# tzjtatata/Myriad

Hardware: AMD Instinct MI355X
Metric: images/sec fine-tune step (Vicuna-7B + LoRA-style adapters, 224px) (higher is better)
Workload: dtype bf16

## Files before the change

include/myriad_hip.h:

```cpp
#ifndef MYRIAD_HIP_H
#define MYRIAD_HIP_H
#include <stdint.h>

#ifdef __cplusplus
extern "C" {
#endif

typedef struct ihipStream_t* mh_stream_t;

#define MH_OK 0
#define MH_ERR_ARG (-1)
#define MH_ERR_LAUNCH (-2)
#define MH_ERR_UNSUPPORTED (-3)

#define MH_GEMM_OUT_F32 1
#define MH_GEMM_GELU 2
#define MH_GEMM_REGSTAGE 4

int mh_gemm_bf16_nt(const void* A, int lda, const void* B, int ldb, void* C, int ldc, int M, int N, int K,
                    const float* bias, const float* residual, int ldr, int flags, float alpha, mh_stream_t s);

int mh_gemm_plan(int M, int N, int K, int flags, int* kernel, int* splits);

int mh_prof_start(int capacity, mh_stream_t s);
// ... 57 lines not shown
long mh_layernorm_param_grads_ws_floats(int M, int D);
int mh_layernorm_param_grads(const float* dy, const float* x, float* dgamma, float* dbeta, int M, int D, float eps,
                             int accumulate, float p_out, unsigned long long seed_out, float* ws, long ws_floats,
                             mh_stream_t s);
int mh_layernorm_fwd_dropout(const float* z, const float* res, const float* w, const float* b, float* x_out, void* y_bf16,
                             float* y_f32, int M, int D, float eps, float p_in, unsigned long long seed_in, float p_out,
                             unsigned long long seed_out, mh_stream_t s);
int mh_layernorm_bwd_dropout(const float* dy, const float* x, const float* w, float* dx, void* dz_bf16, int M, int D,
                             float eps, float p_in, unsigned long long seed_in, float p_out, unsigned long long seed_out,
                             mh_stream_t s);
int mh_dropout_keep_mask(float* out, long n, float p, unsigned long long seed, mh_stream_t s);
long mh_gemm_tn_wgrad_ws_floats(int M, int N, int K, int splits);
int mh_gemm_tn_wgrad_auto_splits(int M, int N, int K);
int mh_gemm_tn_wgrad(const void* dy, long lddy, const void* x, long ldx, float* out, long ldo, float* bias, int M, int N, int K,
                     int accumulate, int splits, float* ws, long ws_floats, mh_stream_t s);

int mh_rope_inplace(void* x, int ld, int col0, int n_tok, int n_heads, int head_dim, const int* pos,
                    const float* cos_tab, const float* sin_tab, float sign, mh_stream_t s);
int mh_silu_mul_fwd(const void* gu, void* h, int M, int I, mh_stream_t s);
int mh_silu_mul_bwd(const void* dh, const void* gu, void* dgu, int M, int I, mh_stream_t s);
int mh_silu_mul_fwd_blk(const void* gu, void* h, int M, int I, int blk, mh_stream_t s);
int mh_silu_mul_bwd_blk(const void* dh, const void* gu, void* dgu, int M, int I, int blk, mh_stream_t s);
int mh_gemm_swiglu_fwd(const void* X, int ldx, const void* Wgu, int ldw, void* gu, int ldgu, void* act, int ldact, int M,
                       int I, int K, mh_stream_t s);
int mh_gemm_swiglu_bwd(const void* dH, int lddh, const void* WdT, int ldw, const void* gu, int ldgu, void* dgu, int lddgu,
                       void* dact_buf, int M, int I, int K, mh_stream_t s);
int mh_gelu_fwd(const void* x, void* y, long n, mh_stream_t s);
int mh_gelu_bwd(const void* dy, const void* x, void* dx, long n, mh_stream_t s);
int mh_gemm_gelu_fwd(const void* X, int ldx, const void* W, int ldw, const float* bias, void* pre, int ldpre, void* act, int ldact,
                     int M, int N, int K, mh_stream_t s);
// ... 205 lines not shown
                        const void* eroded, int y0s, int x0s, int dy0, int dx0, int h, int w, const double* Sh, const double* cy,
                        const double* Sw, const double* cx, double* ws, int mixed, mh_stream_t s);

int mh_adamw_gated(float* p, const float* g, float* m, float* v, long n, double lr, double beta1, double beta2, double eps,
                   double weight_decay, double grad_scale, const float* used, const int* steps, mh_stream_t s);
int mh_adamw_bump(const float* used, int* steps, int n, mh_stream_t s);

long mh_grad_sumsq_slots(long n);
int mh_grad_sumsq(const float* g, long n, const float* used, double* partials, long slots, mh_stream_t s);
int mh_clip_rank_sum(const double* partials, long n_partials, double* rank_sums, int world, int rank, mh_stream_t s);
int mh_clip_finalize(const double* partials, long n_partials, const double* rank_sums, int world, double max_norm,
                     double grad_scale, int guard, double* ctl, mh_stream_t s);
int mh_adamw_gated_ctl(float* p, const float* g, float* m, float* v, long n, double lr, double beta1, double beta2, double eps,
                       double weight_decay, const float* used, const int* steps, const double* ctl, mh_stream_t s);
int mh_adamw_bump_ctl(const float* used, int* steps, int n, const double* ctl, mh_stream_t s);

int mh_l2norm_rows(const float* x, long ldx, void* y_bf16, float* y_f32, long ldy, int M, int D, float eps, mh_stream_t s);
int mh_pair_logits(const float* p, long ldp, const float* text, float* out, long rows, int rows_per_batch, int C, float scale,
                   mh_stream_t s);
int mh_zs_accumulate(const float* logits, float* mask_acc, float* map_acc, int B, int h, int S, float w, mh_stream_t s);
int mh_rowmax_skip(const float* scores, long lds, float* acc, long rows, int cols, int period, float w, mh_stream_t s);
int mh_bilinear_ac(const float* in, float* out, int B, int h, int w, int H, int W, int one_minus, mh_stream_t s);

int mh_bank_sim_chunk_rows(void);
int mh_bank_sim_max(const void* q, long q_row0, long q_sample_rows, const void* bank, const int* bank_off, const int* bank_rows,
                    float* part, int B, int L, int D, int max_chunks, mh_stream_t s);
int mh_bank_sim_finish(const float* part, const int* bank_rows, float* sim, float* simmask, float* amap, int T, int B,
                       int max_chunks, int h, int S, float w, mh_stream_t s);

long mh_mask_components_lds_bytes(int H, int W);
// ... 37 lines not shown
```

myriad_amd/csrc/optim.hip:

```cpp
#include "common.h"

__global__ void adamw_kernel(float* __restrict__ p, const float* __restrict__ g, float* __restrict__ m,
                             float* __restrict__ v, bf16_t* __restrict__ shadow, long n4, float lr, float beta1,
                             float beta2, float omb1, float omb2, float eps, float wd, float bc1, float bc2_sqrt,
                             float gscale) {
  for (long it = blockIdx.x * (long)blockDim.x + threadIdx.x; it < n4; it += (long)gridDim.x * blockDim.x) {
    float4_t pp = *reinterpret_cast<const float4_t*>(p + it * 4);
    const float4_t gg = *reinterpret_cast<const float4_t*>(g + it * 4);
    float4_t mm = *reinterpret_cast<const float4_t*>(m + it * 4);
    float4_t vv = *reinterpret_cast<const float4_t*>(v + it * 4);
#pragma unroll
    for (int e = 0; e < 4; ++e) {
      const float gr = gg[e] * gscale;
      pp[e] *= (1.f - lr * wd);
      mm[e] = beta1 * mm[e] + omb1 * gr;
      vv[e] = beta2 * vv[e] + omb2 * gr * gr;
      const float denom = sqrtf(vv[e]) / bc2_sqrt + eps;
      pp[e] -= (lr / bc1) * (mm[e] / denom);
    }
    *reinterpret_cast<float4_t*>(p + it * 4) = pp;
    *reinterpret_cast<float4_t*>(m + it * 4) = mm;
    *reinterpret_cast<float4_t*>(v + it * 4) = vv;
    if (shadow) {
      uint2 pk;
// ... 218 lines not shown
  if (ctl[2] != 0.0 && i < n && used[i] > 0.f) steps[i] += 1;
}

extern "C" int mh_adamw_gated_ctl(float* p, const float* g, float* m, float* v, long n, double lr, double beta1, double beta2,
                                  double eps, double weight_decay, const float* used, const int* steps, const double* ctl,
                                  hipStream_t stream) {
  if (n < 0 || n % 4 || !used || !steps || !ctl || (n > 0 && (!p || !g || !m || !v))) return MH_ERR_ARG;
  if (n == 0) return MH_OK;
  long grid = (n / 4 + 255) / 256;
  if (grid > 256 * 16) grid = 256 * 16;
  hipLaunchKernelGGL(adamw_gated_ctl_kernel, dim3((int)grid), dim3(256), 0, stream, p, g, m, v, n / 4, (float)lr, beta1, beta2,
                     (float)eps, (float)weight_decay, used, steps, ctl);
  MH_CHECK_LAUNCH();
  return MH_OK;
}
extern "C" int mh_adamw_bump_ctl(const float* used, int* steps, int n, const double* ctl, hipStream_t stream) {
  if (n <= 0) return MH_OK;
  if (!used || !steps || !ctl) return MH_ERR_ARG;
  hipLaunchKernelGGL(adamw_bump_ctl_kernel, dim3((n + 63) / 64), dim3(64), 0, stream, used, steps, n, ctl);
  MH_CHECK_LAUNCH();
  return MH_OK;
}
```

myriad_amd/csrc/wgrad.hip:

```cpp
#include "common.h"

#define TN_BN 64
#define TN_BK 64
#define TN_BM 32
#define TN_RS (TN_BK + 16)
typedef __attribute__((address_space(3))) short4_t tn_lds_s4;

__device__ __forceinline__ short8_t tn_frag(const bf16_t* img, int jd, int lr, int lg) {
  const bf16_t* p = img + (4 * lg + (lr >> 2)) * TN_RS + 16 * jd + 4 * (lr & 3);
  const short4_t a = __builtin_amdgcn_ds_read_tr16_b64_v4i16((tn_lds_s4*)p);
  const short4_t b = __builtin_amdgcn_ds_read_tr16_b64_v4i16((tn_lds_s4*)(p + 16 * TN_RS));
  return (short8_t){a[0], a[1], a[2], a[3], b[0], b[1], b[2], b[3]};
}

__global__ __launch_bounds__(256) void gemm_tn_wgrad_kernel(const bf16_t* __restrict__ dy, long lddy, const bf16_t* __restrict__ x,
                                                            long ldx, float* out, long ldo, float* bias, float* ws, float* wsb,
                                                            int M, int N, int K, int rows_per, int accumulate) {
  __shared__ __attribute__((aligned(16))) bf16_t img[2][TN_BM * TN_RS];
  __shared__ float red[TN_BM][TN_BN + 1];
  const int tid = threadIdx.x, lane = tid & 63, wave = tid >> 6, lr = lane & 15, lg = lane >> 4;
  const int k0 = blockIdx.x * TN_BK, n0 = blockIdx.y * TN_BN, z = blockIdx.z;
  const int m0 = z * rows_per;
  const int m1 = min(M, m0 + rows_per);
  const bool want_bias = bias != nullptr && blockIdx.x == 0;
// ... 109 lines not shown
  rows_per = (rows_per + TN_BM - 1) / TN_BM * TN_BM;
  if (rows_per == 0) rows_per = TN_BM;
  float* wsb = splits > 1 ? ws + (long)splits * N * K : nullptr;
  hipLaunchKernelGGL(gemm_tn_wgrad_kernel, dim3(K / TN_BK, N / TN_BN, splits), dim3(256), 0, stream, (const bf16_t*)dy, lddy,
                     (const bf16_t*)x, ldx, out, ldo, bias, ws, wsb, M, N, K, rows_per, accumulate);
  MH_CHECK_LAUNCH();
  if (splits > 1) {
    const long n4 = (long)N * (K / 4);
    hipLaunchKernelGGL(tn_split_reduce_kernel, dim3((unsigned)((n4 + 255) / 256)), dim3(256), 0, stream, ws, wsb, splits, out,
                       ldo, bias, N, K, accumulate);
    MH_CHECK_LAUNCH();
  }
  return MH_OK;
}

#define LNP_NT 256
#define LNP_NW 4
#define LNP_ROWS 16
#define LNP_IT 4

__global__ __launch_bounds__(LNP_NT) void layernorm_param_partial_kernel(const float* __restrict__ dy, const float* __restrict__ x,
                                                                         float* __restrict__ part, int M, int D, float eps,
                                                                         float p_out, unsigned long long seed_out) {
  __shared__ float red[LNP_NW];
  const int r0 = blockIdx.x * LNP_ROWS, r1 = min(M, r0 + LNP_ROWS);
  float4_t sg[LNP_IT], sb[LNP_IT];
#pragma unroll
  for (int c = 0; c < LNP_IT; ++c) sg[c] = sb[c] = (float4_t){0.f, 0.f, 0.f, 0.f};
  for (int row = r0; row < r1; ++row) {
    const float* xr = x + (size_t)row * D;
// ... 83 lines not shown
```

myriad_amd/myriad.py:

```python
from __future__ import annotations

import numbers
import os
import random
from collections import OrderedDict
from typing import Dict, List, Optional, Tuple

import torch
import torch.nn as nn

from . import _lib, ops
from .eva_vit import EvaViTHIP
from .llama import LlamaHIP
from .networks import LoraAdaptor, VENet, from_reference_layout, to_reference_layout, ve_param_specs
from .qformer import QFormerHIP, qformer_param_specs
from .registry import registry

BF16, F32 = torch.bfloat16, torch.float32


def uses_weight_decay(name: str, ndim: int) -> bool:
    return not (ndim < 2 or "bias" in name or "ln" in name or "bn" in name)


# ... 97 lines not shown
        self.steps_dev = torch.zeros(max(nm, 1), dtype=torch.int32, device=self.dev)
        self.flat_m = torch.zeros(off, dtype=F32, device=self.dev)
        self.flat_v = torch.zeros(off, dtype=F32, device=self.dev)
        self.p, self.g = {}, {}
        self.ref_shape = {}
        for name, ishape, rshape in self.specs:
            o, n = self.offsets[name]
            self.p[name] = self.flat_p[o:o + n].view(ishape)
            self.g[name] = self.flat_g[o:o + n].view(ishape)
            self.ref_shape[name] = rshape
        self.ctl = None
        self._norm_ws = None
        self._rank_sums = None
        self.step = 0
        self.version = 0

    def n_params(self) -> int:
        return sum(n for _, n in self.offsets.values())

    def mark_used(self, used_modules) -> None:
        if not self.modules:
            return
        flags = torch.tensor([1.0 if m in used_modules else 0.0 for m in self.modules], dtype=F32)
        self.used.copy_(ops.h2d(flags, self.dev))

    def module_steps(self) -> Dict[str, int]:
        st = self.steps_dev.cpu().tolist()
        return {m: int(st[i]) for i, m in enumerate(self.modules)}

    def set_module_steps(self, steps: Dict[str, int]) -> None:
# ... 2 lines not shown

    def module_range(self, module: str, decays: bool = True):
        if module not in self.modules:
            return None
        mi = self.modules.index(module)
        for m2, a, b, d in self.ranges:
            if m2 == mi and d == decays:
                return a, b
        return None

    def adamw_module(self, module: str, lr: float, weight_decay: float = 0.05, beta2: float = 0.999) -> None:
        mi = self.modules.index(module)
        self.version += 1
        for m2, a, b, decays in self.ranges:
            if m2 == mi:
                ops.adamw_gated(self.flat_p[a:b], self.flat_g[a:b], self.flat_m[a:b], self.flat_v[a:b], lr,
                                weight_decay if decays else 0.0, self.used[mi:mi + 1], self.steps_dev[mi:mi + 1], beta2=beta2)

    def adamw_pieces(self, pieces, lr: float, weight_decay: float = 0.05, beta2: float = 0.999, grad_scale: float = 1.0) -> None:
        self.version += 1
        for mi, a0, b0, decays in self.ranges:
            for lo, hi in pieces:
                a, b = max(a0, lo), min(b0, hi)
                if a < b:
                    ops.adamw_gated(self.flat_p[a:b], self.flat_g[a:b], self.flat_m[a:b], self.flat_v[a:b], lr,
                                    weight_decay if decays else 0.0, self.used[mi:mi + 1], self.steps_dev[mi:mi + 1], beta2=beta2,
                                    grad_scale=grad_scale)

    def adamw_step(self, lr: float, weight_decay: float = 0.05, beta2: float = 0.999, grad_scale: float = 1.0, shard=None,
                   skip=(), exclude=(), clip=None):
        self.step += 1
        self.version += 1
        pieces = None
        if shard is not None:
            pieces = [tuple(shard)] if isinstance(shard[0], int) else [tuple(p) for p in shard]
            if sum(hi - lo for lo, hi in pieces) < self.total:
                self.moments_complete = False
        skip_idx = {self.modules.index(m) for m in skip if m in self.modules}
        todo = update_pieces(self.ranges, pieces, exclude, skip_idx)
        if clip is not None:
            self._prepare_clip(todo, grad_scale, clip)
        for mi, a, b, decays in todo:
            if clip is None:
                ops.adamw_gated(self.flat_p[a:b], self.flat_g[a:b], self.flat_m[a:b], self.flat_v[a:b], lr,
                                weight_decay if decays else 0.0, self.used[mi:mi + 1], self.steps_dev[mi:mi + 1], beta2=beta2,
                                grad_scale=grad_scale)
            else:
                ops.adamw_gated_ctl(self.flat_p[a:b], self.flat_g[a:b], self.flat_m[a:b], self.flat_v[a:b], lr,
                                    weight_decay if decays else 0.0, self.used[mi:mi + 1], self.steps_dev[mi:mi + 1], self.ctl,
                                    beta2=beta2)
        if self.modules:
            if clip is None:
                ops.adamw_bump(self.used, self.steps_dev)
            else:
                ops.adamw_bump_ctl(self.used, self.steps_dev, self.ctl)

    def _prepare_clip(self, todo, grad_scale: float, clip) -> None:
        if self.ctl is None:
            self.ctl = torch.zeros(4, dtype=torch.float64, device=self.dev)
        need = sum(ops.grad_sumsq_slots(b - a) for _, a, b, _ in todo)
        if self._norm_ws is None or self._norm_ws.numel() < need:
            whole = sum(ops.grad_sumsq_slots(b - a) for _, a, b, _ in self.ranges)
            self._norm_ws = torch.zeros(max(need, whole) + 64, dtype=torch.float64, device=self.dev)
        ws, off = self._norm_ws, 0
        for mi, a, b, _ in todo:
# ... 31 lines not shown
            fan_in = cin * k * k
        bound = 1.0 / math.sqrt(fan_in)
        return (torch.rand(rshape) * 2 - 1) * bound
    raise KeyError(f"{name}: not in the weight files and no constructor init exists (load it with `ckpt`)")


class _LossBridge(torch.autograd.Function):

    @staticmethod
    def forward(ctx, anchor, model, loss):
        ctx.model = model
        return loss.detach().clone()

    @staticmethod
    def backward(ctx, gout):
        ctx.model.backward(float(gout), accumulate=ctx.model._grads_live())
        return None, None, None


class MyriadHIP(nn.Module):
    arch = "myriad"

    def __init__(self, weights, cfg: Optional[dict] = None, device="cuda:0"):
        super().__init__()
        cfg = dict(cfg or {})
        self.cfg = cfg
        self._dev = torch.device(device)
        self.max_txt_len = cfg.get("max_txt_len", 160)
        self.end_sym = cfg.get("end_sym", "###")
        self.k_shot = cfg.get("k_shot", 0)
# ... 56 lines not shown
        self._params = OrderedDict()
        for name, ishape, rshape in self.store.specs:
            if name in lora_init and name not in weights:
                src = lora_init[name]
            elif name in weights:
                src = weights[name]
            else:
                src = init_trainable(name, rshape)
            self.store.p[name].copy_(from_reference_layout(src.to(self._dev, F32), ishape))
            prm = nn.Parameter(self.store.p[name], requires_grad=True)
            prm.grad = self.store.g[name]
            self._params[name] = prm
            self._register_dotted(name, prm)
        if self.arch == "myriad":
            self.adaptor = LoraAdaptor(self.store.p, self.store.g)
            self.ve_tok = VENet("VETokenizer.", 5, self.Dl, self.store.p, self.store.g, self._dev)
            self.ve_ins = VENet("VEInstructor.", 1, self.Dq, self.store.p, self.store.g, self._dev)
        if self.use_lora:
            self.lora = LoraQV(len(self.llama.layers), self.Dl, int(cfg.get("lora_r", 8)),
                               float(cfg.get("lora_alpha", 16)), float(cfg.get("lora_dropout", 0.05)),
                               self.store.p, self.store.g, self._dev)
            self.lora.base_seed = int(cfg.get("lora_dropout_seed", torch.initial_seed())) & ((1 << 31) - 1)
            self.llama.attach_lora(self.lora)
        if self.train_qformer:
            self.query_tokens_f32 = self.store.p["query_tokens"]
            self.qformer.bind_trainable(self.store, need_denc=self.arch == "myriad" or self.train_vit)
        if self.train_vit:
            self.ln_w, self.ln_b = self.store.p["ln_vision.weight"], self.store.p["ln_vision.bias"]
            self.vit.bind_trainable(self.store, need_backward=need_bwd)
        self._pending_update = None
        self._vit_stream, self._vit_prefetched = None, None
# ... 42 lines not shown
    def merged_lora_state_dict(self) -> "OrderedDict[str, torch.Tensor]":
        if not self.use_lora:
            raise ValueError("merged_lora_state_dict: no LoRA is attached (cfg use_lora)")
        from .lora import merged_qv_names
        self.finish_update()
        out, D = OrderedDict(), self.Dl
        for i, L in enumerate(self.llama.layers):
            m = self.lora.merge_layer(i, L, "rows")
            nq, nv = merged_qv_names(i)
            out[nq], out[nv] = m[:D].clone(), m[2 * D:].clone()
        return out

    def load_state_dict(self, sd, strict: bool = False):
        self.finish_update()
        self.store.version += 1
        missing = []
        for name, ishape, _ in self.store.specs:
            if name in sd:
                self.store.p[name].copy_(from_reference_layout(sd[name].to(self._dev, F32), ishape))
            else:
                missing.append(name)
        if self.train_vit:
            self.vit.refresh()
        else:
            self._load_vision_keys(sd)
        if strict and missing:
            raise KeyError(missing)
        return missing

    @torch.no_grad()
# ... 243 lines not shown
        if c is None:
            raise RuntimeError("backward() without a training forward")
        head = None
        if accumulate and float(gscale) == 1.0 and self.arch == "myriad" and self.ve_tok.head_accumulates_in_place:
            o_n = self.store.offsets.get("VETokenizer.meta_net.15.weight")
            if o_n is not None and o_n[1] >= (1 << 20):
                head = (o_n[0], o_n[0] + o_n[1])
        self._acc_head = head
        fg = self.store.flat_g_comm
        if not accumulate:
            prev = None
        elif head is None:
            prev = fg.clone()
        else:
            prev = (fg[:head[0]].clone(), fg[head[1]:].clone())
        zeroed, self._g_zeroed = getattr(self, "_g_zeroed", None), None
        if zeroed is not None and not accumulate:
            torch.cuda.current_stream().wait_event(zeroed)
        elif head is None:
            fg.zero_()
        else:
            fg[:head[0]].zero_()
            fg[head[1]:].zero_()
        used = {"lora"} if self.use_lora else set()
        if self.arch == "myriad":
            used.add("expert_adaptor")
            if c["use_tok"]:
                used.add("VETokenizer")
            if c["use_ins"]:
                used.add("VEInstructor")
        else:
            used.add("llama_proj")
        if self.train_qformer:
            used.add("Qformer")
        if self.train_vit:
            used.update(("visual_encoder", "ln_vision"))
        self.store.mark_used(used)
        self._bridge_used = (self._bridge_used | used) if accumulate else set(used)
# ... 65 lines not shown
            else:
                self.ve_ins.backward(dins)
        dy = self._ln_vision_backward(denc, c)
        dx = self.adaptor.backward(dy, need_dx=self.train_vit)
        if self.train_vit:
            self.vit.backward(dx.view(B, c["N"], self.Dv), grads=self.vit.grad_views)
        if self.llama.lora is not None:
            self.llama.lora.join_wgrads()
        if leaf_ev is not None:
            torch.cuda.current_stream().wait_event(leaf_ev)
        if ins_ev is not None:
            torch.cuda.current_stream().wait_event(ins_ev)
        del leaf_keep, ins_keep
        self._finish_backward()

    def _ln_vision_backward(self, denc: torch.Tensor, c) -> torch.Tensor:
        d2 = denc.view(c["B"] * c["N"], self.Dv)
        if self.train_vit:
            ops.layernorm_param_grads(d2, c["y"], 1e-5, self.store.g["ln_vision.weight"], self.store.g["ln_vision.bias"])
        return ops.layernorm_bwd(d2, c["y"], self.ln_w, 1e-5)[0]

    def _query_tokens_grad(self, dq: torch.Tensor) -> None:
        B, nq, D = dq.shape
        self.store.g["query_tokens"].view(-1).copy_(ops.colsum(dq.reshape(B, nq * D)[:, :self.nq0 * D]))

    def _start_early_exchange(self, early_exchange) -> None:
        dp, k = early_exchange[0], early_exchange[1]
        st = self.store
        if len(early_exchange) > 2 and getattr(dp, "supports_early_update", False):
            lr, wd, beta2 = early_exchange[2]

            def then():
                st.adamw_pieces(dp.part_shards(st.total, k), lr, wd, beta2=beta2, grad_scale=1.0 / dp.world)
                dp.gather_part(st.flat_p, k)
            dp.start_part(st.flat_g_comm, st.total, k, then=then)
        else:
            dp.start_part(st.flat_g_comm, st.total, k)

    def _finish_backward(self):
        if self._bwd_gscale != 1.0:
            ops.scale_(self.store.flat_g, self._bwd_gscale)
        if self._bwd_prev is not None:
            fg = self.store.flat_g_comm
            if isinstance(self._bwd_prev, tuple):
                a, b = self._acc_head
                for pv, dst in ((self._bwd_prev[0], fg[:a]), (self._bwd_prev[1], fg[b:])):
                    if pv.numel():
                        ops.copy2d(pv.view(1, -1), dst.view(1, -1), accumulate=True)
            else:
# ... 112 lines not shown
            vit_out = self._take_prefetched_vit(samples)
            if next_samples is not None:
                self.prefetch_vit(next_samples)
            if self._pending_update is not None and vit_out is not None:
                self.finish_update()
            elif self._pending_update is not None and self.train_vit:
                self.finish_update()
            elif self._pending_update is not None:
                vit_out = self.vit.forward(self._image_of(samples))
                self.finish_update()
            if (self._accum_count == 0 and self._leaf_aside and self._dev.type == "cuda"
                    and os.environ.get("MYRIAD_EARLY_ZERO", "1") != "0"):
                aux, main = self._side_stream("leaf"), torch.cuda.current_stream()
                aux.wait_stream(main)
                with torch.cuda.stream(aux):
                    self.store.flat_g_comm.zero_()
                    self._g_zeroed = torch.cuda.Event()
                    self._g_zeroed.record(aux)
            try:
                loss = self._forward_impl(samples, True, vit_out=vit_out)
            except Exception:
                self._g_zeroed = None
                raise
            accumulate = self._accum_count > 0
            due = accum_update_due(self._accum_count + 1, accum_grad_iters, accum_index)
            early = (lr, weight_decay, beta2) if (due and not accumulate and (dp is None or dp.world == 1) and allreduce is None
                                                  and world == 1 and clip is None
                                                  and os.environ.get("MYRIAD_EARLY_ADAMW", "1") != "0") else None
            if dp is not None and dp.world > 1 and self.arch == "myriad" and hasattr(dp, "set_segments"):
                self._dp_segment(dp)
            early_x = None
            if (dp is not None and dp.world > 1 and overlap and due and not accumulate and self.arch == "myriad"
                    and hasattr(dp, "start_part") and os.environ.get("MYRIAD_DP_EARLY", "1") != "0"):
                k = self._dp_segment(dp)
                if k is not None:
                    early_upd = clip is None and os.environ.get("MYRIAD_DP_EARLY_ADAMW", "1") != "0"
# ... 6 lines not shown
            if dp is not None and dp.world > 1 and overlap:
                dp.start(self.store.flat_g_comm, self.store.total)
                self._pending_update = (dp, lr, weight_decay, beta2, clip)
            else:
                shard = None
                if dp is not None and dp.world > 1:
                    dp.allreduce(self.store.flat_g_comm, self.store.total)
                    shard = self._dp_shards(dp)
                elif allreduce is not None:
                    allreduce(self.store.flat_g_comm)
                    world = max(world, 1)
                self.store.adamw_step(lr, weight_decay, beta2=beta2, grad_scale=1.0 / (dp.world if dp is not None else world),
                                      shard=shard, skip=self._early_done, clip=clip.for_dp(dp) if clip is not None else None)
                if shard is not None:
                    dp.gather_params(self.store.flat_p)
        return loss

    def _dp_shards(self, dp):
        if getattr(dp, "mode", "allreduce") != "rs_ag":
            return None
        return dp.shards(self.store.total) if hasattr(dp, "shards") else [dp.shard(self.store.total)[:2]]

    def _dp_segment(self, dp):
        if getattr(self, "_dp_seg_of", None) is not None and self._dp_seg_of[0] is dp:
            return self._dp_seg_of[1]
        k = None
        rng = self.store.module_range("VETokenizer", True)
        if rng is not None:
            a, b = ops.round_up(rng[0], 32), rng[1] // 32 * 32
            if b - a >= (1 << 20):
# ... 6 lines not shown
    def finish_update(self):
        if self._pending_update is not None:
            dp, lr, wd, beta2, clip = self._pending_update
            self._pending_update = None
            if dp is None:
                self.store.adamw_step(lr, wd, beta2=beta2, clip=clip)
                return
            dp.wait()
            shard = self._dp_shards(dp)
            done = dp.take_early_done() if hasattr(dp, "take_early_done") else set()
            segs = dp.segments(self.store.total) if done else []
            self.store.adamw_step(lr, wd, beta2=beta2, grad_scale=1.0 / dp.world, shard=shard, exclude=[segs[k] for k in done],
                                  clip=clip.for_dp(dp) if clip is not None else None)
            if shard is not None:
                dp.gather_params(self.store.flat_p, skip=done) if done else dp.gather_params(self.store.flat_p)

    def grad_stats(self) -> dict:
        return self.store.grad_stats()

    def _generate_args(self, generate_kwargs) -> dict:
        kw = dict(generate_kwargs)
        stops = kw.pop("stop_ids", None)
        crit = kw.pop("stopping_criteria", None)
        if crit is not None:
            stops = [tuple(int(t) for t in torch.as_tensor(st).reshape(-1).tolist()) for c in crit for st in getattr(c, "stops", [])]
        if stops is None:
            stops = ()
        max_new = kw.pop("max_new_tokens", None)
        if max_new is None:
            max_len = kw.pop("max_length", None)
# ... 291 lines not shown
```

myriad_amd/networks.py:

```python
from __future__ import annotations

from typing import Dict, List, Optional, Tuple

import torch

from . import ops

BF16, F32 = torch.bfloat16, torch.float32

STEM_CH = [(1, 4), (4, 16), (16, 64), (64, 256), (256, 1024)]
STEM_IDX = (0, 3, 6, 9, 12)


def ve_param_specs(prefix: str, head_out: int, head_k: int) -> List[Tuple[str, Tuple[int, ...], Tuple[int, ...]]]:
    specs = []
    for idx, (ci, co) in zip(STEM_IDX, STEM_CH):
        specs.append((f"{prefix}meta_net.{idx}.weight", (co, 9 * ci), (co, ci, 3, 3)))
        specs.append((f"{prefix}meta_net.{idx}.bias", (co,), (co,)))
    specs.append((f"{prefix}meta_net.15.weight", (head_out, head_k * head_k * 1024), (head_out, 1024, head_k, head_k)))
    specs.append((f"{prefix}meta_net.15.bias", (head_out,), (head_out,)))
    return specs


def from_reference_layout(t: torch.Tensor, internal_shape) -> torch.Tensor:
    if t.dim() == 4 and len(internal_shape) != 4:
        return t.permute(0, 2, 3, 1).reshape(internal_shape).contiguous()
    return t.reshape(internal_shape).contiguous()


def to_reference_layout(t: torch.Tensor, ref_shape) -> torch.Tensor:
    if len(ref_shape) == 4 and t.dim() != 4:
        co, ci, kh, kw = ref_shape
        return t.reshape(co, kh, kw, ci).permute(0, 3, 1, 2).contiguous()
    return t.reshape(ref_shape).contiguous()


class VENet:

    def __init__(self, prefix: str, head_k: int, head_out: int, params: Dict[str, torch.Tensor],
                 grads: Dict[str, torch.Tensor], device):
        self.prefix, self.head_k, self.head_out = prefix, head_k, head_out
        self.p, self.g, self.dev = params, grads, torch.device(device)
        self._saved = None

    def _w(self, idx):
        return self.p[f"{self.prefix}meta_net.{idx}.weight"], self.p[f"{self.prefix}meta_net.{idx}.bias"]

    def forward(self, maps: torch.Tensor, save_for_backward: bool = True) -> torch.Tensor:
        B, _, H, W = maps.shape
        x = ops.to_bf16(maps.contiguous()).view(B, H, W, 1)
        saved = []
        for idx, (ci, co) in zip(STEM_IDX, STEM_CH):
            wm, bias = self._w(idx)
            wp = ops.conv_pack(wm, bias)
            col = ops.im2col(x, 3, 3, 1)
            y = ops.gemm(col, wp, out_dtype=F32)
            saved.append((col, y, wp, H, W, ci, co))
            x = ops.relu_pool_fwd(y, B, H, W, co)
            H, W = H // 2, W // 2
        wm, bias = self._w(15)
        if self.head_k == 1:
            x2 = x.view(B * H * W, 1024)
            wb = ops.to_bf16(wm)
            out = ops.gemm(x2, wb, bias=bias, out_dtype=F32)
            head = (x2, wb, None, True)
            T = H * W
        else:
            k = self.head_k
            T = (H - k + 1) * (W - k + 1)
            if wm.shape[1] % 64 == 0:
                wp = ops.to_bf16(wm)
                col = ops.im2col(x, k, k, 0, bias_col=False)
                out = ops.gemm(col, wp, bias=bias, out_dtype=F32)
                head = (col, wp, (H, W), True)
            else:
                wp = ops.conv_pack(wm, bias)
                col = ops.im2col(x, k, k, 0)
                out = ops.gemm(col, wp, out_dtype=F32)
                head = (col, wp, (H, W), False)
        if save_for_backward:
            self._saved = dict(stem=saved, head=head, B=B)
        return out.view(B, T, self.head_out)

    @property
    def head_accumulates_in_place(self) -> bool:
        return self.head_k != 1 and (self.head_k * self.head_k * 1024) % 64 == 0

    def backward(self, dtokens: torch.Tensor, accumulate_head: bool = False) -> None:
        sv = self._saved
        if sv is None:
            raise RuntimeError("backward() without saved forward")
        B = sv["B"]
        dy32 = dtokens.reshape(-1, self.head_out).contiguous()
        dyb = ops.to_bf16(dy32)
        gw, gb = self.g[f"{self.prefix}meta_net.15.weight"], self.g[f"{self.prefix}meta_net.15.bias"]
        a, wq, hw = sv["head"][:3]
        dyT = ops.transpose_to_bf16(dyb, 64)
        if self.head_k == 1:
            ops.gemm_auto_f32(dyT, ops.transpose_to_bf16(a, 64), gw)
            gb.copy_(ops.colsum(dy32))
            dp = ops.gemm(dyb, ops.transpose_to_bf16(wq, 64), out_dtype=F32)
        else:
            Kpad = wq.shape[1]
            if sv["head"][3]:
                if accumulate_head:
                    ops.gemm(dyT, ops.transpose_to_bf16(a, 64), out=gw, residual=gw)
                else:
                    ops.gemm_auto_f32(dyT, ops.transpose_to_bf16(a, 64), gw)
                gb.copy_(ops.colsum(dy32))
            else:
                dwp = torch.empty((self.head_out, Kpad), dtype=F32, device=self.dev)
                ops.gemm_auto_f32(dyT, ops.transpose_to_bf16(a, 64), dwp)
                ops.conv_unpack_grad(dwp, gw, gb)
            dcol = ops.gemm(dyb, ops.transpose_to_bf16(wq, 64))
            H, W = hw
            dp = ops.col2im(dcol, B, H, W, 1024, self.head_k, self.head_k, 0)
        for li in range(4, -1, -1):
            col, y, wp, H, W, ci, co = sv["stem"][li]
            idx = STEM_IDX[li]
            dy, dyfull = ops.relu_pool_bwd(dp, y, B, H, W, co, pad_cols_to=64)
            dwp = torch.empty((co, wp.shape[1]), dtype=F32, device=self.dev)
            ops.gemm_auto_f32(ops.transpose_to_bf16(dy, 64), ops.transpose_to_bf16(col, 64), dwp)
            ops.conv_unpack_grad(dwp, self.g[f"{self.prefix}meta_net.{idx}.weight"],
                                 self.g[f"{self.prefix}meta_net.{idx}.bias"])
            if li > 0:
                wpT = ops.transpose_to_bf16(wp, 64)
                dcol = ops.gemm(dyfull, wpT)
                dp = ops.col2im(dcol, B, H, W, ci, 3, 3, 1)
        self._saved = None


# ... 19 lines not shown
```

myriad_amd/ops.py:

```python
from __future__ import annotations

import math
import numbers
from typing import Optional

import os

import torch

from . import _lib

BF16 = torch.bfloat16
F32 = torch.float32

GEMM_OUT_F32 = 1
GEMM_GELU = 2
GEMM_REGSTAGE = 4
GEMM_VARIANT = 0


def _L():
    return _lib.load()


# ... 762 lines not shown
                  accumulate: bool = False, splits: int = 0):
    _chk2d(dy, BF16, "dy")
    _chk2d(x, BF16, "x")
    M, N = dy.shape
    K = x.shape[1]
    if x.shape[0] != M or out.dtype != F32 or out.dim() != 2 or tuple(out.shape) != (N, K) or out.stride(1) != 1:
        raise ValueError(f"gemm_tn_wgrad: dy {tuple(dy.shape)} x {tuple(x.shape)} out {tuple(out.shape)} {out.dtype}")
    if bias is not None and (bias.dtype != F32 or bias.numel() != N or not bias.is_contiguous()):
        raise ValueError("gemm_tn_wgrad: bias must be contiguous f32 [N]")
    L = _L()
    s = int(splits) if splits else L.mh_gemm_tn_wgrad_auto_splits(M, N, K)
    n = L.mh_gemm_tn_wgrad_ws_floats(M, N, K, s)
    ws = torch.empty((n,), dtype=F32, device=dy.device) if n > 0 else None
    _lib.check(L.mh_gemm_tn_wgrad(_p(dy), dy.stride(0), _p(x), x.stride(0), _p(out), out.stride(0), _p(bias), M, N, K,
                                  int(accumulate), s, _p(ws), n, _s()), f"mh_gemm_tn_wgrad M={M} N={N} K={K}")
    return out


def rope_(x2d: torch.Tensor, col0: int, n_heads: int, head_dim: int, pos: torch.Tensor, cos, sin, sign: float = 1.0):
    n_tok = x2d.shape[0]
    _lib.check(_L().mh_rope_inplace(_p(x2d), x2d.stride(0), col0, n_tok, n_heads, head_dim, _p(pos), _p(cos), _p(sin),
                                    float(sign), _s()), "mh_rope_inplace")
    return x2d


def silu_mul_fwd(gu: torch.Tensor):
    M, I2 = gu.shape
    h = torch.empty((M, I2 // 2), dtype=BF16, device=gu.device)
    _lib.check(_L().mh_silu_mul_fwd(_p(gu), _p(h), M, I2 // 2, _s()), "mh_silu_mul_fwd")
    return h
# ... 661 lines not shown
        raise _lib.MyriadHipError("clip_finalize: f64 partials / ctl[4] expected")
    _lib.check(_L().mh_clip_finalize(_p(partials), int(n_partials), _p(rank_sums), 0 if rank_sums is None else rank_sums.numel(),
                                     float("inf") if max_norm is None else float(max_norm), float(grad_scale), int(bool(guard)),
                                     _p(ctl), _s()), "mh_clip_finalize")


def adamw_gated_ctl(p, g, m, v, lr, wd, used: torch.Tensor, steps: torch.Tensor, ctl: torch.Tensor, beta1=0.9, beta2=0.999, eps=1e-8):
    _lib.check(_L().mh_adamw_gated_ctl(_p(p), _p(g), _p(m), _p(v), p.numel(), float(lr), float(beta1), float(beta2), float(eps),
                                       float(wd), _p(used), _p(steps), _p(ctl), _s()), "mh_adamw_gated_ctl")


def adamw_bump_ctl(used: torch.Tensor, steps: torch.Tensor, ctl: torch.Tensor):
    _lib.check(_L().mh_adamw_bump_ctl(_p(used), _p(steps), steps.numel(), _p(ctl), _s()), "mh_adamw_bump_ctl")


def l2norm_rows(x: torch.Tensor, want_bf16: bool = True, want_f32: bool = False, eps: float = 1e-12):
    _chk2d(x, F32, "l2norm_rows.x")
    M, D = x.shape
    yb = torch.empty((M, D), dtype=BF16, device=x.device) if want_bf16 else None
    yf = torch.empty((M, D), dtype=F32, device=x.device) if want_f32 else None
    _lib.check(_L().mh_l2norm_rows(_p(x), x.stride(0), _p(yb), _p(yf), D, M, D, float(eps), _s()), "mh_l2norm_rows")
    return yb, yf


def pair_logits(p: torch.Tensor, text: torch.Tensor, rows_per_batch: int, scale: float = 100.0):
    _chk2d(p, F32, "pair_logits.p")
    rows, C = p.shape
    out = torch.empty((rows, 2), dtype=F32, device=p.device)
    _lib.check(_L().mh_pair_logits(_p(p), p.stride(0), _p(text.contiguous()), _p(out), rows, rows_per_batch, C, float(scale),
                                   _s()), "mh_pair_logits")
# ... 157 lines not shown
```

Measured before the change: 204.4.

## Keep a bf16 shadow of the tokenizer head weight and add a direct head dgrad kernel

The AdamW kernel gains a variant that writes a bf16 copy of one bound parameter range while it updates the fp32 weights, so the tokenizer head no longer needs a separate to_bf16 cast every forward. A dedicated MFMA kernel computes the head's input gradient straight from dy and the untransposed weight, replacing the transpose plus generic GEMM, and the weight gradient is written directly by the TN wgrad kernel. The gradient-zeroing pass also skips that head's slice when the head overwrites it in place. The cost is extra shadow-validity bookkeeping: it must be invalidated on backward, on load_state_dict and after DP gathers, and any missed invalidation would feed stale weights to the forward pass.

```diff
diff --git a/include/myriad_hip.h b/include/myriad_hip.h
--- a/include/myriad_hip.h
+++ b/include/myriad_hip.h
@@ -95,6 +95,8 @@
 int mh_gemm_tn_wgrad_auto_splits(int M, int N, int K);
 int mh_gemm_tn_wgrad(const void* dy, long lddy, const void* x, long ldx, float* out, long ldo, float* bias, int M, int N, int K,
                      int accumulate, int splits, float* ws, long ws_floats, mh_stream_t s);
+
+int mh_head_dgrad(const void* dy, long lddy, const void* w, long ldw, void* out, long ldo, int M, int N, int K, mh_stream_t s);
 
 int mh_rope_inplace(void* x, int ld, int col0, int n_tok, int n_heads, int head_dim, const int* pos,
                     const float* cos_tab, const float* sin_tab, float sign, mh_stream_t s);
@@ -330,6 +332,12 @@
 int mh_adamw_gated_ctl(float* p, const float* g, float* m, float* v, long n, double lr, double beta1, double beta2, double eps,
                        double weight_decay, const float* used, const int* steps, const double* ctl, mh_stream_t s);
 int mh_adamw_bump_ctl(const float* used, int* steps, int n, const double* ctl, mh_stream_t s);
+int mh_adamw_gated_shadow(float* p, const float* g, float* m, float* v, long n, double lr, double beta1, double beta2, double eps,
+                          double weight_decay, double grad_scale, const float* used, const int* steps, void* shadow_bf16,
+                          long shadow_lo, long shadow_n, mh_stream_t s);
+int mh_adamw_gated_ctl_shadow(float* p, const float* g, float* m, float* v, long n, double lr, double beta1, double beta2,
+                              double eps, double weight_decay, const float* used, const int* steps, const double* ctl,
+                              void* shadow_bf16, long shadow_lo, long shadow_n, mh_stream_t s);
 
 int mh_l2norm_rows(const float* x, long ldx, void* y_bf16, float* y_f32, long ldy, int M, int D, float eps, mh_stream_t s);
 int mh_pair_logits(const float* p, long ldp, const float* text, float* out, long rows, int rows_per_batch, int C, float scale,
diff --git a/myriad_amd/csrc/optim.hip b/myriad_amd/csrc/optim.hip
--- a/myriad_amd/csrc/optim.hip
+++ b/myriad_amd/csrc/optim.hip
@@ -256,6 +256,86 @@
   MH_CHECK_LAUNCH();
   return MH_OK;
 }
+template <bool CTL>
+__global__ void adamw_gated_shadow_kernel(float* __restrict__ p, const float* __restrict__ g, float* __restrict__ m,
+                                          float* __restrict__ v, long n4, float lr, double beta1_d, double beta2_d, float eps,
+                                          float wd, float gscale_arg, const float* __restrict__ used,
+                                          const int* __restrict__ steps, const double* __restrict__ ctl,
+                                          bf16_t* __restrict__ shadow, long s_lo4, long s_hi4) {
+  if (CTL) {
+    if (ctl[2] == 0.0 || *used <= 0.f) return;
+  } else {
+    if (*used <= 0.f) return;
+  }
+  const float gscale = CTL ? (float)ctl[0] : gscale_arg;
+  const double st = (double)(*steps + 1);
+  const float bc1 = (float)(1.0 - pow(beta1_d, st));
+  const float bc2_sqrt = (float)sqrt(1.0 - pow(beta2_d, st));
+  const float omb1 = (float)(1.0 - beta1_d), omb2 = (float)(1.0 - beta2_d);
+  const float beta1 = (float)beta1_d, beta2 = (float)beta2_d;
+  for (long it = blockIdx.x * (long)blockDim.x + threadIdx.x; it < n4; it += (long)gridDim.x * blockDim.x) {
+    float4_t pp = *reinterpret_cast<const float4_t*>(p + it * 4);
+    const float4_t gg = *reinterpret_cast<const float4_t*>(g + it * 4);
+    float4_t mm = *reinterpret_cast<const float4_t*>(m + it * 4);
+    float4_t vv = *reinterpret_cast<const float4_t*>(v + it * 4);
+#pragma unroll
+    for (int e = 0; e < 4; ++e) {
+      const float gr = gg[e] * gscale;
+      pp[e] *= (1.f - lr * wd);
+      mm[e] = beta1 * mm[e] + omb1 * gr;
+      vv[e] = beta2 * vv[e] + omb2 * gr * gr;
+      const float denom = sqrtf(vv[e]) / bc2_sqrt + eps;
+      pp[e] -= (lr / bc1) * (mm[e] / denom);
+    }
+    *reinterpret_cast<float4_t*>(p + it * 4) = pp;
+    *reinterpret_cast<float4_t*>(m + it * 4) = mm;
+    *reinterpret_cast<float4_t*>(v + it * 4) = vv;
+    if (it >= s_lo4 && it < s_hi4) {
+      uint2 pk;
+      pk.x = pack_bf2(pp[0], pp[1]);
+      pk.y = pack_bf2(pp[2], pp[3]);
+      *reinterpret_cast<uint2*>(shadow + (it - s_lo4) * 4) = pk;
+    }
+  }
+}
+
+static inline bool shadow_args_ok(const void* shadow, long n, long shadow_lo, long shadow_n) {
+  if (shadow_n == 0) return true;
+  return shadow && shadow_lo >= 0 && shadow_n > 0 && shadow_lo % 4 == 0 && shadow_n % 4 == 0 && shadow_lo + shadow_n <= n &&
+         ((uintptr_t)shadow & 7) == 0;
+}
+
+extern "C" int mh_adamw_gated_shadow(float* p, const float* g, float* m, float* v, long n, double lr, double beta1,
+                                     double beta2, double eps, double weight_decay, double grad_scale, const float* used,
+                                     const int* steps, void* shadow_bf16, long shadow_lo, long shadow_n, hipStream_t stream) {
+  if (n < 0 || n % 4 || !used || !steps || (n > 0 && (!p || !g || !m || !v))) return MH_ERR_ARG;
+  if (!shadow_args_ok(shadow_bf16, n, shadow_lo, shadow_n)) return MH_ERR_ARG;
+  if (n == 0) return MH_OK;
+  long grid = (n / 4 + 255) / 256;
+  if (grid > 256 * 16) grid = 256 * 16;
+  hipLaunchKernelGGL(adamw_gated_shadow_kernel<false>, dim3((int)grid), dim3(256), 0, stream, p, g, m, v, n / 4, (float)lr,
+                     beta1, beta2, (float)eps, (float)weight_decay, (float)grad_scale, used, steps, (const double*)nullptr,
+                     (bf16_t*)shadow_bf16, shadow_lo / 4, (shadow_lo + shadow_n) / 4);
+  MH_CHECK_LAUNCH();
+  return MH_OK;
+}
+
+extern "C" int mh_adamw_gated_ctl_shadow(float* p, const float* g, float* m, float* v, long n, double lr, double beta1,
+                                         double beta2, double eps, double weight_decay, const float* used, const int* steps,
+                                         const double* ctl, void* shadow_bf16, long shadow_lo, long shadow_n,
+                                         hipStream_t stream) {
+  if (n < 0 || n % 4 || !used || !steps || !ctl || (n > 0 && (!p || !g || !m || !v))) return MH_ERR_ARG;
+  if (!shadow_args_ok(shadow_bf16, n, shadow_lo, shadow_n)) return MH_ERR_ARG;
+  if (n == 0) return MH_OK;
+  long grid = (n / 4 + 255) / 256;
+  if (grid > 256 * 16) grid = 256 * 16;
+  hipLaunchKernelGGL(adamw_gated_shadow_kernel<true>, dim3((int)grid), dim3(256), 0, stream, p, g, m, v, n / 4, (float)lr,
+                     beta1, beta2, (float)eps, (float)weight_decay, 1.f, used, steps, ctl, (bf16_t*)shadow_bf16, shadow_lo / 4,
+                     (shadow_lo + shadow_n) / 4);
+  MH_CHECK_LAUNCH();
+  return MH_OK;
+}
+
 extern "C" int mh_adamw_bump_ctl(const float* used, int* steps, int n, const double* ctl, hipStream_t stream) {
   if (n <= 0) return MH_OK;
   if (!used || !steps || !ctl) return MH_ERR_ARG;
diff --git a/myriad_amd/csrc/wgrad.hip b/myriad_amd/csrc/wgrad.hip
--- a/myriad_amd/csrc/wgrad.hip
+++ b/myriad_amd/csrc/wgrad.hip
@@ -147,6 +147,90 @@
   return MH_OK;
 }
 
+#define HD_BK 64
+#define HD_ROWS 128
+#define HD_AS (HD_ROWS + 8)
+#define HD_MAXM 128
+
+__global__ __launch_bounds__(256) void head_dgrad_kernel(const bf16_t* __restrict__ dy, long lddy, const bf16_t* __restrict__ w,
+                                                         long ldw, bf16_t* __restrict__ out, long ldo, int M, int N) {
+  __shared__ __attribute__((aligned(16))) bf16_t wimg[HD_ROWS * TN_RS];
+  __shared__ __attribute__((aligned(16))) bf16_t aimg[HD_MAXM * HD_AS];
+  const int tid = threadIdx.x, lane = tid & 63, wave = tid >> 6, lr = lane & 15, lg = lane >> 4;
+  const int k0 = blockIdx.x * HD_BK;
+  const int mt = (M + 15) >> 4;
+  const short8_t zero8 = (short8_t){0, 0, 0, 0, 0, 0, 0, 0};
+  for (int i = tid; i < HD_MAXM * HD_AS / 8; i += 256) reinterpret_cast<short8_t*>(aimg)[i] = zero8;
+  const int srow = tid >> 3, scol = (tid & 7) * 8;
+  const int arow = tid >> 4, acol = (tid & 15) * 8;
+  short8_t rw[4], ra[8];
+  auto load_step = [&](int nb) {
+#pragma unroll
+    for (int i = 0; i < 4; ++i) {
+      const int n = nb + srow + 32 * i;
+      rw[i] = zero8;
+      if (n < N) rw[i] = *reinterpret_cast<const short8_t*>(w + (long)n * ldw + k0 + scol);
+    }
+#pragma unroll
+    for (int c = 0; c < 8; ++c) {
+      const int r = arow + 16 * c;
+      ra[c] = zero8;
+      if (c < mt && r < M && nb + acol < N) ra[c] = *reinterpret_cast<const short8_t*>(dy + (long)r * lddy + nb + acol);
+    }
+  };
+  float4_t acc[8];
+#pragma unroll
+  for (int t = 0; t < 8; ++t) acc[t] = (float4_t){0.f, 0.f, 0.f, 0.f};
+  load_step(0);
+  for (int nb = 0; nb < N; nb += HD_ROWS) {
+    __syncthreads();
+#pragma unroll
+    for (int i = 0; i < 4; ++i) *reinterpret_cast<short8_t*>(&wimg[(srow + 32 * i) * TN_RS + scol]) = rw[i];
+#pragma unroll
+    for (int c = 0; c < 8; ++c) {
+      const int r = arow + 16 * c;
+      if (c < mt && r < M) *reinterpret_cast<short8_t*>(&aimg[r * HD_AS + acol]) = ra[c];
+    }
+    __syncthreads();
+    if (nb + HD_ROWS < N) load_step(nb + HD_ROWS);
+#pragma unroll 1
+    for (int s = 0; s < HD_ROWS / TN_BM; ++s) {
+      const short8_t b = tn_frag(wimg + s * TN_BM * TN_RS, wave, lr, lg);
+#pragma unroll
+      for (int t = 0; t < 8; ++t) {
+        if (t < mt) {
+          const bf16_t* ap = aimg + (16 * t + lr) * HD_AS + TN_BM * s + 4 * lg;
+          const short4_t a0 = *reinterpret_cast<const short4_t*>(ap);
+          const short4_t a1 = *reinterpret_cast<const short4_t*>(ap + 16);
+          const short8_t a = (short8_t){a0[0], a0[1], a0[2], a0[3], a1[0], a1[1], a1[2], a1[3]};
+          acc[t] = __builtin_amdgcn_mfma_f32_16x16x32_bf16(a, b, acc[t], 0, 0, 0);
+        }
+      }
+    }
+  }
+#pragma unroll
+  for (int t = 0; t < 8; ++t) {
+    if (t < mt) {
+#pragma unroll
+      for (int e = 0; e < 4; ++e) {
+        const int r = 16 * t + 4 * lg + e;
+        if (r < M) out[(long)r * ldo + k0 + 16 * wave + lr] = f2bf(acc[t][e]);
+      }
+    }
+  }
+}
+
+extern "C" int mh_head_dgrad(const void* dy, long lddy, const void* w, long ldw, void* out, long ldo, int M, int N, int K,
+                             hipStream_t stream) {
+  if (M <= 0 || M > HD_MAXM || N <= 0 || K <= 0 || N % 8 || K % HD_BK || lddy % 8 || ldw % 8 || lddy < N || ldw < K || ldo < K)
+    return MH_ERR_ARG;
+  if (!dy || !w || !out || (((uintptr_t)dy | (uintptr_t)w) & 15)) return MH_ERR_ARG;
+  hipLaunchKernelGGL(head_dgrad_kernel, dim3(K / HD_BK), dim3(256), 0, stream, (const bf16_t*)dy, lddy, (const bf16_t*)w, ldw,
+                     (bf16_t*)out, ldo, M, N);
+  MH_CHECK_LAUNCH();
+  return MH_OK;
+}
+
 #define LNP_NT 256
 #define LNP_NW 4
 #define LNP_ROWS 16
diff --git a/myriad_amd/myriad.py b/myriad_amd/myriad.py
--- a/myriad_amd/myriad.py
+++ b/myriad_amd/myriad.py
@@ -135,6 +135,54 @@
         self._rank_sums = None
         self.step = 0
         self.version = 0
+        self._shadow = None
+        self._shadow_ok, self._shadow_pver, self._shadow_armed = False, -1, False
+
+    def bind_shadow(self, name: str) -> None:
+        o, n = self.offsets[name]
+        if o % 4 or n % 4:
+            raise ValueError(f"bind_shadow({name}): offset and size must be multiples of 4")
+        self._shadow = (name, o, o + n, torch.empty(self.p[name].shape, dtype=torch.bfloat16, device=self.dev))
+        self._shadow_ok = self._shadow_armed = False
+
+    def invalidate_shadow(self) -> None:
+        self._shadow_ok = self._shadow_armed = False
+
+    def _shadow_holds_cast(self) -> bool:
+        return self._shadow is not None and self._shadow_ok and self.flat_p._version == self._shadow_pver
+
+    @property
+    def shadow_current(self) -> bool:
+        return self._shadow_holds_cast() and self._shadow_armed
+
+    def _shadow_cast(self) -> None:
+        ops.to_bf16(self.p[self._shadow[0]], out=self._shadow[3])
+        self._shadow_ok, self._shadow_pver = True, self.flat_p._version
+
+    def shadow_operand(self, name: str):
+        if self._shadow is None or self._shadow[0] != name:
+            return None
+        if not self.shadow_current:
+            self._shadow_cast()
+        self._shadow_armed = False
+        return self._shadow[3]
+
+    def _adamw_range(self, mi: int, a: int, b: int, lr: float, wd: float, beta2: float, grad_scale: float = 1.0, ctl=None) -> None:
+        args = (self.flat_p[a:b], self.flat_g[a:b], self.flat_m[a:b], self.flat_v[a:b], lr, wd, self.used[mi:mi + 1],
+                self.steps_dev[mi:mi + 1])
+        sh = self._shadow
+        if sh is not None and a <= sh[1] and sh[2] <= b:
+            if not self._shadow_holds_cast():
+                self._shadow_cast()
+            ops.adamw_gated_shadow(*args, sh[3].view(-1), sh[1] - a, ctl=ctl, beta2=beta2, grad_scale=grad_scale)
+            self._shadow_armed = True
+            return
+        if sh is not None and a < sh[2] and sh[1] < b:
+            self.invalidate_shadow()
+        if ctl is None:
+            ops.adamw_gated(*args, beta2=beta2, grad_scale=grad_scale)
+        else:
+            ops.adamw_gated_ctl(*args, ctl, beta2=beta2)
 
     def n_params(self) -> int:
         return sum(n for _, n in self.offsets.values())
@@ -167,8 +215,7 @@
         self.version += 1
         for m2, a, b, decays in self.ranges:
             if m2 == mi:
-                ops.adamw_gated(self.flat_p[a:b], self.flat_g[a:b], self.flat_m[a:b], self.flat_v[a:b], lr,
-                                weight_decay if decays else 0.0, self.used[mi:mi + 1], self.steps_dev[mi:mi + 1], beta2=beta2)
+                self._adamw_range(mi, a, b, lr, weight_decay if decays else 0.0, beta2)
 
     def adamw_pieces(self, pieces, lr: float, weight_decay: float = 0.05, beta2: float = 0.999, grad_scale: float = 1.0) -> None:
         self.version += 1
@@ -176,9 +223,7 @@
             for lo, hi in pieces:
                 a, b = max(a0, lo), min(b0, hi)
                 if a < b:
-                    ops.adamw_gated(self.flat_p[a:b], self.flat_g[a:b], self.flat_m[a:b], self.flat_v[a:b], lr,
-                                    weight_decay if decays else 0.0, self.used[mi:mi + 1], self.steps_dev[mi:mi + 1], beta2=beta2,
-                                    grad_scale=grad_scale)
+                    self._adamw_range(mi, a, b, lr, weight_decay if decays else 0.0, beta2, grad_scale)
 
     def adamw_step(self, lr: float, weight_decay: float = 0.05, beta2: float = 0.999, grad_scale: float = 1.0, shard=None,
                    skip=(), exclude=(), clip=None):
@@ -194,14 +239,8 @@
         if clip is not None:
             self._prepare_clip(todo, grad_scale, clip)
         for mi, a, b, decays in todo:
-            if clip is None:
-                ops.adamw_gated(self.flat_p[a:b], self.flat_g[a:b], self.flat_m[a:b], self.flat_v[a:b], lr,
-                                weight_decay if decays else 0.0, self.used[mi:mi + 1], self.steps_dev[mi:mi + 1], beta2=beta2,
-                                grad_scale=grad_scale)
-            else:
-                ops.adamw_gated_ctl(self.flat_p[a:b], self.flat_g[a:b], self.flat_m[a:b], self.flat_v[a:b], lr,
-                                    weight_decay if decays else 0.0, self.used[mi:mi + 1], self.steps_dev[mi:mi + 1], self.ctl,
-                                    beta2=beta2)
+            self._adamw_range(mi, a, b, lr, weight_decay if decays else 0.0, beta2, grad_scale,
+                              ctl=None if clip is None else self.ctl)
         if self.modules:
             if clip is None:
                 ops.adamw_bump(self.used, self.steps_dev)
@@ -263,6 +302,7 @@
 
     @staticmethod
     def backward(ctx, gout):
+        ctx.model.store.invalidate_shadow()
         ctx.model.backward(float(gout), accumulate=ctx.model._grads_live())
         return None, None, None
 
@@ -349,7 +389,8 @@
             self._register_dotted(name, prm)
         if self.arch == "myriad":
             self.adaptor = LoraAdaptor(self.store.p, self.store.g)
-            self.ve_tok = VENet("VETokenizer.", 5, self.Dl, self.store.p, self.store.g, self._dev)
+            self.store.bind_shadow("VETokenizer.meta_net.15.weight")
+            self.ve_tok = VENet("VETokenizer.", 5, self.Dl, self.store.p, self.store.g, self._dev, store=self.store)
             self.ve_ins = VENet("VEInstructor.", 1, self.Dq, self.store.p, self.store.g, self._dev)
         if self.use_lora:
             self.lora = LoraQV(len(self.llama.layers), self.Dl, int(cfg.get("lora_r", 8)),
@@ -422,6 +463,7 @@
     def load_state_dict(self, sd, strict: bool = False):
         self.finish_update()
         self.store.version += 1
+        self.store.invalidate_shadow()
         missing = []
         for name, ishape, _ in self.store.specs:
             if name in sd:
@@ -695,14 +737,23 @@
             prev = fg.clone()
         else:
             prev = (fg[:head[0]].clone(), fg[head[1]:].clone())
+        over = None
+        if not accumulate and float(gscale) == 1.0 and c["use_tok"]:
+            over = self._head_grad_range()
         zeroed, self._g_zeroed = getattr(self, "_g_zeroed", None), None
+        left, self._g_head_left = getattr(self, "_g_head_left", None), None
         if zeroed is not None and not accumulate:
             torch.cuda.current_stream().wait_event(zeroed)
-        elif head is None:
-            fg.zero_()
-        else:
+            if left is not None and over is None:
+                fg[left[0]:left[1]].zero_()
+        elif head is not None:
             fg[:head[0]].zero_()
             fg[head[1]:].zero_()
+        elif over is not None:
+            fg[:over[0]].zero_()
+            fg[over[1]:].zero_()
+        else:
+            fg.zero_()
         used = {"lora"} if self.use_lora else set()
         if self.arch == "myriad":
             used.add("expert_adaptor")
@@ -798,6 +849,14 @@
         del leaf_keep, ins_keep
         self._finish_backward()
 
+    def _head_grad_range(self):
+        if self.arch != "myriad" or not self.ve_tok.head_accumulates_in_place:
+            return None
+        o_n = self.store.offsets.get("VETokenizer.meta_net.15.weight")
+        if o_n is None or o_n[1] < (1 << 20):
+            return None
+        return o_n[0], o_n[0] + o_n[1]
+
     def _ln_vision_backward(self, denc: torch.Tensor, c) -> torch.Tensor:
         d2 = denc.view(c["B"] * c["N"], self.Dv)
         if self.train_vit:
@@ -817,6 +876,7 @@
             def then():
                 st.adamw_pieces(dp.part_shards(st.total, k), lr, wd, beta2=beta2, grad_scale=1.0 / dp.world)
                 dp.gather_part(st.flat_p, k)
+                st.invalidate_shadow()
             dp.start_part(st.flat_g_comm, st.total, k, then=then)
         else:
             dp.start_part(st.flat_g_comm, st.total, k)
@@ -959,12 +1019,20 @@
                 aux, main = self._side_stream("leaf"), torch.cuda.current_stream()
                 aux.wait_stream(main)
                 with torch.cuda.stream(aux):
-                    self.store.flat_g_comm.zero_()
+                    left = self._head_grad_range()
+                    fg = self.store.flat_g_comm
+                    if left is None:
+                        fg.zero_()
+                    else:
+                        fg[:left[0]].zero_()
+                        fg[left[1]:].zero_()
+                    self._g_head_left = left
                     self._g_zeroed = torch.cuda.Event()
                     self._g_zeroed.record(aux)
             try:
                 loss = self._forward_impl(samples, True, vit_out=vit_out)
             except Exception:
+                self._g_head_left = None
                 self._g_zeroed = None
                 raise
             accumulate = self._accum_count > 0
@@ -1001,6 +1069,7 @@
                                       shard=shard, skip=self._early_done, clip=clip.for_dp(dp) if clip is not None else None)
                 if shard is not None:
                     dp.gather_params(self.store.flat_p)
+                    self.store.invalidate_shadow()
         return loss
 
     def _dp_shards(self, dp):
@@ -1037,6 +1106,7 @@
                                   clip=clip.for_dp(dp) if clip is not None else None)
             if shard is not None:
                 dp.gather_params(self.store.flat_p, skip=done) if done else dp.gather_params(self.store.flat_p)
+                self.store.invalidate_shadow()
 
     def grad_stats(self) -> dict:
         return self.store.grad_stats()
diff --git a/myriad_amd/networks.py b/myriad_amd/networks.py
--- a/myriad_amd/networks.py
+++ b/myriad_amd/networks.py
@@ -38,9 +38,10 @@
 class VENet:
 
     def __init__(self, prefix: str, head_k: int, head_out: int, params: Dict[str, torch.Tensor],
-                 grads: Dict[str, torch.Tensor], device):
+                 grads: Dict[str, torch.Tensor], device, store=None):
         self.prefix, self.head_k, self.head_out = prefix, head_k, head_out
         self.p, self.g, self.dev = params, grads, torch.device(device)
+        self.store = store
         self._saved = None
 
     def _w(self, idx):
@@ -69,7 +70,9 @@
             k = self.head_k
             T = (H - k + 1) * (W - k + 1)
             if wm.shape[1] % 64 == 0:
-                wp = ops.to_bf16(wm)
+                wp = self.store.shadow_operand(f"{self.prefix}meta_net.15.weight") if self.store is not None else None
+                if wp is None:
+                    wp = ops.to_bf16(wm)
                 col = ops.im2col(x, k, k, 0, bias_col=False)
                 out = ops.gemm(col, wp, bias=bias, out_dtype=F32)
                 head = (col, wp, (H, W), True)
@@ -95,6 +98,13 @@
         dyb = ops.to_bf16(dy32)
         gw, gb = self.g[f"{self.prefix}meta_net.15.weight"], self.g[f"{self.prefix}meta_net.15.bias"]
         a, wq, hw = sv["head"][:3]
+        if self.head_k != 1 and sv["head"][3] and self.head_out % 64 == 0 and dyb.shape[0] <= 128:
+            ops.gemm_tn_wgrad(dyb, a, gw, accumulate=accumulate_head)
+            gb.copy_(ops.colsum(dy32))
+            dcol = ops.head_dgrad(dyb, wq)
+            H, W = hw
+            dp = ops.col2im(dcol, B, H, W, 1024, self.head_k, self.head_k, 0)
+            return self._backward_stem(dp, sv, B)
         dyT = ops.transpose_to_bf16(dyb, 64)
         if self.head_k == 1:
             ops.gemm_auto_f32(dyT, ops.transpose_to_bf16(a, 64), gw)
@@ -112,9 +122,12 @@
                 dwp = torch.empty((self.head_out, Kpad), dtype=F32, device=self.dev)
                 ops.gemm_auto_f32(dyT, ops.transpose_to_bf16(a, 64), dwp)
                 ops.conv_unpack_grad(dwp, gw, gb)
-            dcol = ops.gemm(dyb, ops.transpose_to_bf16(wq, 64))
+            dcol = ops.gemm(dyb,ops.transpose_to_bf16(wq, 64))
             H, W = hw
             dp = ops.col2im(dcol, B, H, W, 1024, self.head_k, self.head_k, 0)
+        self._backward_stem(dp, sv, B)
+
+    def _backward_stem(self, dp: torch.Tensor, sv, B: int) -> None:
         for li in range(4, -1, -1):
             col, y, wp, H, W, ci, co = sv["stem"][li]
             idx = STEM_IDX[li]
diff --git a/myriad_amd/ops.py b/myriad_amd/ops.py
--- a/myriad_amd/ops.py
+++ b/myriad_amd/ops.py
@@ -800,6 +800,22 @@
     ws = torch.empty((n,), dtype=F32, device=dy.device) if n > 0 else None
     _lib.check(L.mh_gemm_tn_wgrad(_p(dy), dy.stride(0), _p(x), x.stride(0), _p(out), out.stride(0), _p(bias), M, N, K,
                                   int(accumulate), s, _p(ws), n, _s()), f"mh_gemm_tn_wgrad M={M} N={N} K={K}")
+    return out
+
+
+def head_dgrad(dy: torch.Tensor, w: torch.Tensor, out: Optional[torch.Tensor] = None) -> torch.Tensor:
+    _chk2d(dy, BF16, "dy")
+    _chk2d(w, BF16, "w")
+    M, N = dy.shape
+    K = w.shape[1]
+    if w.shape[0] != N:
+        raise ValueError(f"head_dgrad: dy {tuple(dy.shape)} w {tuple(w.shape)}")
+    if out is None:
+        out = torch.empty((M, K), dtype=BF16, device=dy.device)
+    elif out.dtype != BF16 or tuple(out.shape) != (M, K) or out.stride(1) != 1:
+        raise ValueError(f"head_dgrad: out {tuple(out.shape)} {out.dtype}")
+    _lib.check(_L().mh_head_dgrad(_p(dy), dy.stride(0), _p(w), w.stride(0), _p(out), out.stride(0), M, N, K, _s()),
+               f"mh_head_dgrad M={M} N={N} K={K}")
     return out
 
 
@@ -1491,6 +1507,20 @@
     _lib.check(_L().mh_adamw_bump_ctl(_p(used), _p(steps), steps.numel(), _p(ctl), _s()), "mh_adamw_bump_ctl")
 
 
+def adamw_gated_shadow(p, g, m, v, lr, wd, used: torch.Tensor, steps: torch.Tensor, shadow: torch.Tensor, shadow_lo: int = 0,
+                       ctl: Optional[torch.Tensor] = None, beta1=0.9, beta2=0.999, eps=1e-8, grad_scale=1.0):
+    if shadow.dtype != BF16 or not shadow.is_contiguous():
+        raise ValueError("adamw_gated_shadow: shadow must be contiguous bf16")
+    if ctl is None:
+        _lib.check(_L().mh_adamw_gated_shadow(_p(p), _p(g), _p(m), _p(v), p.numel(), float(lr), float(beta1), float(beta2),
+                                              float(eps), float(wd), float(grad_scale), _p(used), _p(steps), _p(shadow),
+                                              int(shadow_lo), shadow.numel(), _s()), "mh_adamw_gated_shadow")
+    else:
+        _lib.check(_L().mh_adamw_gated_ctl_shadow(_p(p), _p(g), _p(m), _p(v), p.numel(), float(lr), float(beta1), float(beta2),
+                                                  float(eps), float(wd), _p(used), _p(steps), _p(ctl), _p(shadow), int(shadow_lo),
+                                                  shadow.numel(), _s()), "mh_adamw_gated_ctl_shadow")
+
+
 def l2norm_rows(x: torch.Tensor, want_bf16: bool = True, want_f32: bool = False, eps: float = 1e-12):
     _chk2d(x, F32, "l2norm_rows.x")
     M, D = x.shape
```

Measured after the change: 205.1, median of 6. No clear change (+0.3%).
